# markokr/libacm

Measured on AMD Instinct MI355X. Metric: decoded PCM Msamples/sec over a batch of ACM streams (hot path on HBM-resident staged input), higher is better.
Workload: dtype int32

## Files before the change

### libacm_amd/capi.py

```python
import ctypes as C
import os

import numpy as np

from . import _build

FMT_S16LE, FMT_S16BE, FMT_U16LE, FMT_U16BE = 0, 1, 2, 3
PLAN_AUTO, PLAN_STAGEWISE = 0, 1
PLAN_FORM_ONLY, PLAN_UPLOAD_ASYNC = 0x100, 0x200
PLAN_LEAN_ALWAYS, PLAN_NO_LEAN, PLAN_FORCE_HALO, PLAN_FORCE_CARRY = 0x400, 0x800, 0x1000, 0x2000
PLAN_EXTRA = 0
BATCH_EXTRA = 0


def batch_ranges(n):
    return (int(n) & 0xFF) << 8
ERR_NO_DEVICE = -101
ERR_ARG = -103
ERR_RANGE = -105


class BlkHdr(C.Structure):
    _fields_ = [("val", C.c_uint32), ("pwr", C.c_uint32)]

# ... 394 lines not shown
    def one(i):
        if ntiles[i]:
            d = descs[i]
            buf = np.empty(cap[i], dtype=np.uint8)
            used = C.c_uint64()
            rc = L.acmhip_mform_rows(d.level, idx[d.idx_off:].ctypes.data, rows[i], buf.ctypes.data, 0, pairs[p_at[i]:].ctypes.data,
                                     C.byref(used))
            if rc == ERR_RANGE:
                ntiles[i] = 0
                return
            _check(rc, "acmhip_mform_rows")
            parts[i] = buf[:(used.value + 63) // 64 * 64]
    with ThreadPoolExecutor(max_workers=max(1, threads)) as ex:
        list(ex.map(one, range(n)))
    total = sum(p.size for p in parts if p is not None)
    if (total >> 6) >= 1 << 30:
        raise AcmHipError("byte-plane arena beyond 64 GB")
    at = 0
    for i in range(n):
        if parts[i] is not None:
            k = int(L.acmhip_mform_pairs(rows[i]))
            pairs[p_at[i]:p_at[i] + k] += np.uint32((at // 64) << 2)
            at += parts[i].size
    data = np.empty(max(at, 16) + 64, dtype=np.uint8)
    at = 0
    for i in range(n):
        if parts[i] is not None:
            data[at:at + parts[i].size] = parts[i]
            at += parts[i].size
    data[at:] = 0
    return MformArena(data, pairs, [PackedStream(p_at[i], ntiles[i], FORM_BYTEPLANE) for i in range(n)])


def mform_unrows(level, blob, pairs, nrows):
    out = np.zeros(nrows << level, dtype=np.int16)
    _check(lib().acmhip_mform_unrows(level, blob.ctypes.data, pairs.ctypes.data, nrows, out.ctypes.data), "acmhip_mform_unrows")
    return out


def pack_streams(idx, descs, threads=1):
    from concurrent.futures import ThreadPoolExecutor
    L = lib()
    n = len(descs)
    ntiles, chunk_off, blob_cap, slots = [0] * n, [0] * n, [0] * n, [0] * n
    c_at = 0
    for i, d in enumerate(descs):
        tr = L.acmhip_packed_tile_rows(d.level)
        if tr > 0 and d.row_begin == 0:
            ntiles[i] = min(d.nrows, d.n_emit >> d.level) // tr
            slots[i] = L.acmhip_packed_slots(d.level)
        chunk_off[i] = c_at
        c_at += ntiles[i] * slots[i]
        if ntiles[i]:
            mb = C.c_uint64()
            _check(L.acmhip_pack_bound(d.level, ntiles[i], C.byref(mb)), "acmhip_pack_bound")
            blob_cap[i] = (mb.value + 15) // 16 * 16
    chunks = np.zeros(max(c_at, 1), dtype=PACKED_CHUNK_DT)
    parts = [None] * n

    def one(i):
        if not ntiles[i]:
            return
        d = descs[i]
        bl = np.zeros(blob_cap[i], dtype=np.uint8)
        nb = C.c_uint64()
        _check(L.acmhip_pack_tiles(d.level, idx[d.idx_off:].ctypes.data, ntiles[i], chunks[chunk_off[i]:].ctypes.data,
# ... 364 lines not shown
```

### libacm_amd/csrc/acm_device.h

```cpp
#ifndef ACM_DEVICE_H
#define ACM_DEVICE_H

#include <stdint.h>

#include "acm_hip.h"

struct AcmDevStream {
	uint64_t idx_off;
	uint64_t hdr_off;
	uint64_t pcm_off;
	uint64_t n_emit;
	uint64_t scratch_off;
	uint32_t level;
	uint32_t rows;
	uint32_t nrows;
	uint32_t row_begin;
	uint32_t halo_row;
	uint32_t pad;
};

struct AcmTile {
	uint32_t stream;
	int32_t row0;
	uint32_t flags;
// ... 81 lines not shown
void acmhip_arena_lock(acmhip_device *dev);
void acmhip_arena_unlock(acmhip_device *dev);
int acmhip_copy_stream(acmhip_device *dev, void **out);
#define ACM_AUX_STREAMS 2
int acmhip_aux_stream(acmhip_device *dev, int k, void **out);
int acmhip_report_hip(int hip_error, const char *what);
void acmhip_set_error_text(const char *text);

#define ACMK_FMT_F32 0x100u
int acmk_tuning_build(void);
int acmk_warmup(void *stream);
int acmk_fused_variants(void);
int acmk_fused_tile_rows(uint32_t level, int variant);
int acmk_fused_has_carry(uint32_t level, int variant);
int acmk_fused_grid(uint32_t level, int variant, int cus);
int acmk_launch_fused(uint32_t level, int variant, int cus, int carry, const AcmDevStream *d_streams, const AcmTile *d_tiles,
		      uint32_t ntiles, const int16_t *d_idx, const acmhip_blkhdr *d_hdr, int16_t *d_pcm, unsigned fmt, void *stream);
int acmk_tile2_rows(uint32_t level);
int acmk_tile2_grid(uint32_t level, int cus);
#define ACM_K2_SINK_BYTES 65536
#define ACM_K2_SINK_F32_BYTES (2 * ACM_K2_SINK_BYTES)
int acmk_launch_tile2(uint32_t level, int cus, const AcmTile2 *d_tiles, uint32_t ntiles, const int16_t *d_idx, const acmhip_blkhdr *d_hdr, int16_t *d_pcm,
		      int16_t *d_sink, unsigned fmt, void *stream);
int acmk_tile2p_rows(uint32_t level);
int acmk_tile2p_group_rows(uint32_t level);
int acmk_tile2p_slots(uint32_t level);
int acmk_tile2p_waves(uint32_t level);
int acmk_tile2p_pad_shift(uint32_t level);
int acmk_launch_tile2p(uint32_t level, int cus, const AcmTile2 *d_tiles, uint32_t ntiles, const acmhip_packed_chunk *d_chunks, const uint8_t *d_blob,
		       const acmhip_blkhdr *d_hdr, int16_t *d_pcm, int16_t *d_sink, unsigned fmt, void *stream);
int acmk_tile2m_rows(uint32_t level);
int acmk_tile2m_lead_in(uint32_t level);
int acmk_tile2m_run_waves(uint32_t level, int cus);
int acmk_tile2m_grid(uint32_t level, int cus);
int acmk_tile2m_stages(uint32_t level);
int acmk_launch_tile2m(uint32_t level, int cus, const AcmTile2 *d_tiles, uint32_t ntiles, const uint8_t *d_mform, const acmhip_mform_pair *d_pairs,
		       const acmhip_blkhdr *d_hdr, int16_t *d_pcm, int16_t *d_sink, unsigned fmt, void *stream);
int acmk_launch_unpack(const AcmDevStream *d_streams, const uint32_t *d_list, uint32_t nlist, uint64_t max_elems,
		       const int16_t *d_idx, const acmhip_blkhdr *d_hdr, int32_t *d_x, uint32_t shift, void *stream);
int acmk_launch_prefix(const AcmDevStream *d_streams, const uint32_t *d_list, uint32_t nlist, uint64_t max_elems,
		       uint32_t level, const int16_t *d_idx, const acmhip_blkhdr *d_hdr, int32_t *d_y, void *stream);
int acmk_plane_tile_rows(void);
int acmk_plane_grid(int cus);
int acmk_launch_fused_plane(int cus, int carry, const AcmDevStream *d_streams, const AcmTile *d_tiles, uint32_t ntiles,
			    const int32_t *d_plane, int16_t *d_pcm, unsigned fmt, void *stream);
int acmk_launch_patch(const AcmDevPatch *d_patches, uint64_t n, int32_t *d_x, void *stream);
int acmk_launch_stage(const AcmDevStream *d_streams, const uint32_t *d_list, uint32_t nlist, uint64_t max_elems,
		      uint32_t level, uint32_t k, const int32_t *d_in, int32_t *d_out, uint32_t shift, void *stream);
int acmk_parse_supported(uint32_t level, uint32_t rows, uint64_t file_len, uint64_t blocks);
int acmk_launch_parse(const AcmParseJob *d_jobs, uint32_t njobs, const uint8_t *d_files, uint32_t *d_colpos, int16_t *d_idx,
		      acmhip_blkhdr *d_hdr, AcmParseResult *d_res, uint32_t *d_flags, uint64_t max_columns, void *stream);
#define ACM_PARSE_RANGE_MAX_STREAMS 32768
int acmk_launch_parse_range(const AcmParseJob *d_jobs, uint32_t njobs, const uint8_t *d_files, uint32_t *d_colpos, int16_t *d_idx,
			    acmhip_blkhdr *d_hdr, AcmParseResult *d_res, uint32_t *d_flags, uint64_t max_columns, uint32_t r, uint32_t R,
			    uint32_t stripes_up, void *stream);
int acmk_launch_parse_range_mf(const AcmParseJob *d_jobs, uint32_t njobs, const uint8_t *d_files, uint32_t *d_colpos, int16_t *d_idx,
			       acmhip_blkhdr *d_hdr, AcmParseResult *d_res, uint32_t *d_flags, uint64_t max_columns, uint32_t r, uint32_t R,
			       uint32_t stripes_up, uint8_t *d_mf, uint32_t *d_pairs, uint32_t *d_blkoff, void *stream);
int acmk_launch_parse_blocks(const AcmParseJob *d_jobs, uint32_t njobs, const AcmBlockJob *d_bjobs, uint32_t nblock, const uint8_t *d_files,
			     uint32_t *d_colpos, int16_t *d_idx, acmhip_blkhdr *d_hdr, AcmParseResult *d_res, uint32_t *d_flags,
			     uint64_t max_columns, void *stream);
uint32_t acmk_stripe_bound(uint32_t file_len, uint32_t s, uint32_t S);
uint32_t acmk_range_bound(uint32_t blocks, uint32_t r, uint32_t R, uint32_t unit);
int acmk_launch_scatter_stripe(const AcmParseJob *d_jobs, uint32_t njobs, const uint64_t *d_stripe_at, const uint8_t *d_stage,
			       uint8_t *d_files, uint32_t s, uint32_t S, void *stream);
int acmk_launch_small(uint32_t level, const AcmDevStream *d_streams, const uint32_t *d_list, uint32_t nlist, uint64_t max_emit,
// ... 21 lines not shown
```

### libacm_amd/csrc/acm_kernels.hip

```cpp
#include <hip/hip_runtime.h>

#include <utility>

#include "acm_device.h"

#ifndef ACM_L14_GROUPS
#define ACM_L14_GROUPS 3, 3, 3, 3, 2
#endif
#ifndef ACM_L13_GROUPS
#define ACM_L13_GROUPS 2, 3, 3, 3, 2
#endif

#ifndef ACM_OUT_F32
#define ACM_OUT_F32 0
#endif
#if ACM_OUT_F32
#define ACM_K_EMIT acm_sw_emit_f32
#define ACM_K_SMALL acm_small_level_f32
#define ACM_K_FUSED acm_fused_tile_f32
#define ACM_K_TILE2 acm_f32_tile2
#define ACM_K_CHUNK acm_f32_chunk
#define ACMK_OUT(name) name##_f32
#else
#define ACM_K_EMIT acm_sw_emit
#define ACM_K_SMALL acm_small_level
#define ACM_K_FUSED acm_fused_tile
#define ACM_K_TILE2 acm_tile2
#define ACM_K_CHUNK acm_chunk
#define ACMK_OUT(name) name
#endif

namespace {

__device__ __forceinline__ uint32_t pcm16(int32_t v, int level, unsigned fmt)
{
	uint32_t w = (uint32_t)(v >> level);
	if (fmt & 2u)
// ... 1979 lines not shown
#define ACM_K3_DPP_HISTORY 1
#endif
	static constexpr bool HISTORY_BY_DPP = ACM_K3_DPP_HISTORY && RR >= 2 && NSW == 2 && RR * SIGMA == 16 && SIGMA >= 4;
	static constexpr bool KEEPS_ROWS = HISTORY_IN_REGISTERS || HISTORY_BY_DPP;
	template <int CTRL, int BANKS>
	static __device__ __forceinline__ v4u_t dpp4(const v4u_t old, const v4u_t src)
	{
		v4u_t r;
#pragma unroll
		for (int v = 0; v < 4; v++)
			r[v] = (uint32_t)__builtin_amdgcn_update_dpp((int)old[v], (int)src[v], CTRL, 0xF, BANKS, false);
		return r;
	}
	static constexpr int DPP_W0_BANKS = (1 << (SIGMA / 4)) - 1;
	static __device__ __forceinline__ void hand_history_on(Raw &raw)
	{
#pragma unroll
		for (int k = 0; k < 2; k++) {
			raw.lo[0][k] = dpp4<0x100 + (16 - SIGMA), DPP_W0_BANKS>(raw.lo[0][k], raw.lo[0][k + NSW]);
			raw.hi[0][k] = dpp4<0x100 + (16 - SIGMA), DPP_W0_BANKS>(raw.hi[0][k], raw.hi[0][k + NSW]);
		}
	}
	static __device__ __forceinline__ void take_history_from_partner(Raw &raw)
	{
#pragma unroll
		for (int k = 0; k < 2; k++) {
			raw.lo[0][k] = dpp4<0x110 + SIGMA, 0xF & ~DPP_W0_BANKS>(raw.lo[0][k], raw.lo[0][k + NSW]);
			raw.hi[0][k] = dpp4<0x110 + SIGMA, 0xF & ~DPP_W0_BANKS>(raw.hi[0][k], raw.hi[0][k + NSW]);
		}
	}
	static constexpr int JM = (TR & 1) ? 1 : TR / 2;
	static_assert(JM + 1 <= NE, "entries in reach are entries fetched");
	static __device__ __forceinline__ uint32_t half_bytes(const uint32_t cls) { return (0x4234u >> (4u * cls)) & 15u; }
	template <int J0>
	static __device__ __forceinline__ uint32_t mode_of(const uint32_t flags, const Desc &d, const uint32_t sval)
	{
		const uint32_t cls = d.e[0] & 3u;
		const uint32_t pair_units = (uint32_t)(COLS / 64) * half_bytes(cls);
		bool ok = (flags & ACM_TILE_ONEBLOCK) != 0 && cls != 0u;
		if constexpr (OutScale<L>::SHIFT != 0)
			ok = ok && sval < 65536u;
#pragma unroll
		for (int j = 1; j <= JM; j++)
			ok = ok && (d.e[j] & 3u) == cls;
#pragma unroll
		for (int j = J0; j < JM; j++)
			ok = ok && (d.e[j + 1] >> 2) - (d.e[j] >> 2) == pair_units;
		return ok ? (cls == ACMHIP_BP_NIB12 ? 3u : cls - (ACMHIP_BP_BYTE - 1u)) : 0u;
	}

#ifndef ACM_K3_LD_MOD
#define ACM_K3_LD_MOD " nt"
#endif
	template <bool KEEP>
	static __device__ __forceinline__ void issue(Raw &raw, const uint8_t *arena, const Desc &d, const int lane, const uint32_t odd, const uint32_t mode)
	{
		static_assert(!KEEP || KEEPS_ROWS, "the rows in front belong to another lane");
		constexpr int K0 = KEEP ? 2 : 0, J0 = KEEP ? 1 : 0;
		const uint32_t i = (uint32_t)lane & 15u, ks = (uint32_t)lane >> 4;
		const uint32_t c = class_of(i), rr = RR == 1 ? 0u : i / SIGMA;
		const uint32_t smode = __builtin_amdgcn_readfirstlane(mode);
		uint32_t va[NX][NG], vh[NX][NG];
		const uint8_t *sb[NX][NG];
		if (mode) {
			const uint32_t hb = smode == 1u ? 2u : smode == 2u ? 4u : 3u;
			const uint64_t base = reinterpret_cast<uint64_t>(arena) + ((uint64_t)(d.e[J0] >> 2) << 6);
			const uint32_t vl = (rr * (uint32_t)(NSW * COLS / 2) + c * (uint32_t)(QN / 2)) * hb + 16u * ks;
			const uint32_t vlh = vl - (smode == 3u ? 8u * ks : 0u);
#pragma unroll
			for (int k = K0; k < NX; k++)
#pragma unroll
				for (int g = 0; g < NG; g++) {
					va[k][g] = vl;
					vh[k][g] = vlh;
					sb[k][g] = sgpr_u64(base + (uint64_t)((((TR & 1 ? odd : 0u) + (uint32_t)(k - K0)) * (uint32_t)(COLS / 2) + group_at(g) * (uint32_t)(QN / 2)) * hb));
				}
		} else {
			const uint32_t e0 = d.e[0];
			const uint8_t *base = sgpr_u64(reinterpret_cast<uint64_t>(arena) + ((uint64_t)(e0 >> 2) << 6));
#pragma unroll
			for (int k = K0; k < NX; k++) {
// ... 53 lines not shown
		for (int g = 0; g < NG; g++)
#pragma unroll
			for (int k = 0; k < 2; k++) {
				raw.lo[g][k] = raw.lo[g][k + NSW];
				raw.hi[g][k] = raw.hi[g][k + NSW];
			}
	}
	static __device__ __forceinline__ void zero_history(Raw &raw)
	{
		const v4u_t z = { 0, 0, 0, 0 };
#pragma unroll
		for (int g = 0; g < NG; g++)
#pragma unroll
			for (int k = 0; k < 2; k++)
				raw.lo[g][k] = raw.hi[g][k] = z;
	}

	static __device__ __forceinline__ v4i_t mfma(const v4u_t data, const v4i_t coef, const v4i_t acc)
	{
		return __builtin_amdgcn_mfma_i32_16x16x64_i8((v4i_t)data, coef, acc, 0, 0, 0);
	}

	static __device__ __forceinline__ int32_t opaque_s(int32_t v)
	{
		asm("" : "+s"(v));
		return v;
	}
	static __device__ __forceinline__ int32_t opaque_v(int32_t v)
	{
		asm("" : "+v"(v));
		return v;
	}

	template <bool WORDS, bool FAST, bool NIB = false>
	static __device__ __forceinline__ void run_t(const Raw &raw, uint32_t *const tile, const Tables &t, const int lane, const uint32_t hvs,
						     const uint32_t in_front, const uint32_t sval, const bool wordu = false, const Desc *dd = nullptr,
						     const uint32_t odd = 0u, const bool nform = false)
	{
		static_assert(!NIB || (WORDS && FAST), "rows in N form are a fast-path matter; the general path takes them to bytes first");
		const v4i_t zero = { 0, 0, 0, 0 };
		const uint32_t h = (uint32_t)lane >> 4, qd = (uint32_t)lane & 15u;
		uint32_t c0[NH], rrd[NH];
		uint32_t o_lane[NH];
#pragma unroll
		for (int hf = 0; hf < NH; hf++) {
			const uint32_t i = 4u * h + (uint32_t)(hf * NVH);
			c0[hf] = RR == 1 ? class_of(i) : i % SIGMA;
			rrd[hf] = RR == 1 ? 0u : i / SIGMA;
			const uint32_t m_lane = rrd[hf] * (uint32_t)(NSW * COLS) + c0[hf] + (uint32_t)SIGMA * qd;
			o_lane[hf] = m_lane + (m_lane >> PS);
		}
		uint32_t bias_at[NSW][NH];
		int32_t val[NSW][NH], dv2[NSW][NH], dv1[NSW][NH];
		bool step2[NSW], step1[NSW];
		bool small[NSW];
#pragma unroll
		for (int s = 0; s < NSW; s++)
			small[s] = OutScale<L>::SHIFT == 0;
		if constexpr (FAST) {
#pragma unroll
			for (int s = 0; s < NSW; s++) {
				step2[s] = step1[s] = false;
				small[s] = true;
#pragma unroll
				for (int hf = 0; hf < NH; hf++)
					val[s][hf] = dv2[s][hf] = dv1[s][hf] = 0;
			}
		} else if constexpr (RR <= 2) {
			int32_t rowval[TR + 2];
#pragma unroll
			for (int k = 0; k < TR + 2; k++)
				rowval[k] = (int32_t)__builtin_amdgcn_readlane(hvs, k);
// ... 36 lines not shown
					dv1[s][hf] = g[s] - g[s + 1];
					if (!one_val) {
						step2[s] = step2[s] || __builtin_amdgcn_ballot_w64(dv2[s][hf] != 0) != 0;
						step1[s] = step1[s] || __builtin_amdgcn_ballot_w64(dv1[s][hf] != 0) != 0;
					}
				}
			}
		}
#pragma unroll
		for (int s = 0; s < NSW; s++)
#pragma unroll
			for (int hf = 0; hf < NH; hf++) {
				const uint32_t row = in_front + rrd[hf] * NSW + s;
				bias_at[s][hf] = ((row < 2 ? row : 2u) * 2u + (c0[hf] == 0 ? 0u : 1u)) * (uint32_t)QN + qd;
			}
		const v4i_t *cf = &t.coef[0][0][lane];
		const auto &hi = raw.hi;
#ifndef ACM_K3_MT_UNROLL
#define ACM_K3_MT_UNROLL 1
#endif
#define ACM_PRAGMA_(x) _Pragma(#x)
#define ACM_UNROLL(n) ACM_PRAGMA_(unroll n)
		ACM_UNROLL(ACM_K3_MT_UNROLL)
		for (int mt = 0; mt < NM; mt++) {
			const v4i_t cf0 = cf[0], cf1 = cf[NM * 64], cf2 = cf[2 * NM * 64];
#pragma unroll
			for (int e = 0; e < NSET; e++) {
				const int g = e / NSW, s = e % NSW;
				int32_t b[NH];
#pragma unroll
				for (int hf = 0; hf < NH; hf++)
					b[hf] = g == 0 ? (&t.bias[0][0][0])[bias_at[s][hf] + 16u * (uint32_t)mt] : 0;
				const v4i_t l1 = mfma(raw.lo[g][s], cf2, zero);
				const v4i_t l2 = mfma(raw.lo[g][s + 1], cf1, l1);
				const v4i_t la = mfma(raw.lo[g][s + 2], cf0, l2);
				v4i_t y;
				if constexpr (FAST) {
					const int32_t sv = opaque_s((int32_t)__builtin_amdgcn_readfirstlane(sval));
#pragma unroll
					for (int v = 0; v < 4; v++)
						y[v] = __mul24(la[v], sv) + (v % NVH == 0 ? b[v / NVH] : 0);
					if constexpr (WORDS) {
						const v4i_t h1 = mfma(hi[g][s], cf2, zero);
						const v4i_t h2 = mfma(hi[g][s + 1], cf1, h1);
						const v4i_t ha = mfma(hi[g][s + 2], cf0, h2);
						if constexpr (NIB) {
							const int32_t sv4 = opaque_s((int32_t)__builtin_amdgcn_readfirstlane(sval << 4));
#pragma unroll
							for (int v = 0; v < 4; v++)
								y[v] = __mul24(ha[v], sv4) + y[v];
						} else {
							const uint32_t sv8 = (uint32_t)opaque_s((int32_t)__builtin_amdgcn_readfirstlane(sval << 8));
#pragma unroll
							for (int v = 0; v < 4; v++)
								y[v] = (int32_t)(__umul24((uint32_t)ha[v], sv8) + (uint32_t)y[v]);
						}
					}
				} else {
#pragma unroll
				for (int v = 0; v < 4; v++)
					y[v] = __mul24(la[v], val[s][v / NVH]) + (v % NVH == 0 ? b[v / NVH] : 0);
				if (step2[s]) {
#pragma unroll
					for (int v = 0; v < 4; v++)
						y[v] += __mul24(l2[v], dv2[s][v / NVH]);
				}
				if (step1[s]) {
#pragma unroll
					for (int v = 0; v < 4; v++)
						y[v] += __mul24(l1[v], dv1[s][v / NVH]);
// ... 47 lines not shown
					}
					if (step1[s]) {
#pragma unroll
						for (int v = 0; v < 4; v++)
							yh[v] += __mul24(h1[v], w1[v / NVH]);
					}
					const uint32_t hs = nform ? 4u : 8u;
#pragma unroll
					for (int v = 0; v < 4; v++)
						y[v] = (int32_t)(((uint32_t)opaque_v(yh[v]) << hs) + (uint32_t)y[v]);
					}
				joined:;
				}
				}
				static_assert(COLS % (1 << PS) == 0 && (SIGMA * 16) % (1 << PS) == 0 &&
					      (NG == 1 || (group_at(NG - 1) % (1 << PS) + CB + 7 < (1 << PS) && SIGMA % (1 << PS) == 0)), "address split");
#pragma unroll
				for (int hf = 0; hf < NH; hf++) {
					uint32_t *const o = tile + (o_lane[hf] + (uint32_t)((s * COLS + ((s * COLS) >> PS)) + (group_at(g) + (group_at(g) >> PS))));
#pragma unroll
					for (int v = 0; v < NVH; v++)
						o[v] = (uint32_t)y[hf * NVH + v];
				}
			}
			cf += 64;
#pragma unroll
			for (int hf = 0; hf < NH; hf++)
				o_lane[hf] += SIGMA * 16 + ((SIGMA * 16) >> PS);
		}
	}

	static __device__ __forceinline__ void run(Raw &raw, uint32_t *const tile, const Tables &t, const int lane_, const uint32_t hvs,
						   const Desc &d, const uint32_t in_front, const uint32_t odd, const uint32_t mode, const uint32_t sval,
						   const bool first)
	{
#ifdef ACM_K3_OPAQUE_LANE
		const int lane = opaque_v(lane_);
#else
		const int lane = lane_;
#endif
		const bool all_new = !KEEPS_ROWS || first;
		if (mode == 3u) {
#pragma unroll
			for (int k = 0; k < NX; k++)
				if (k >= 2 || all_new) {
#pragma unroll
					for (int g = 0; g < NG; g++)
						raw.hi[g][k] = expand_nib(raw.hi[g][k]);
				}
			if constexpr (HISTORY_BY_DPP)
				take_history_from_partner(raw);
			run_t<true, true, true>(raw, tile, t, lane, 0u, in_front, sval);
			return;
		}
		if (mode) {
			if constexpr (HISTORY_BY_DPP)
				take_history_from_partner(raw);
			if (mode == 2u)
				run_t<true, true>(raw, tile, t, lane, 0u, in_front, sval);
			else
				run_t<false, true>(raw, tile, t, lane, 0u, in_front, sval);
			return;
		}
		uint32_t any_word = 0, any_nib = 0, any_wordu = 0;
#pragma unroll
		for (int j = 0; j < NE; j++) {
			any_word |= (d.e[j] & 3u) == ACMHIP_BP_WORD ? 1u : 0u;
			any_nib |= (d.e[j] & 3u) == ACMHIP_BP_NIB12 ? 1u : 0u;
			any_wordu |= (d.e[j] & 3u) == ACMHIP_BP_WORDU ? 1u : 0u;
		}
		any_word |= any_wordu;
		const uint32_t rr = RR == 1 ? 0u : ((uint32_t)lane & 15u) / SIGMA;
		if (any_nib) {
#pragma unroll
// ... 79 lines not shown
		} else if (!(f0 & ACM_TILE_FRESH)) {
			discard = true;
			t--;
		}
	}

	auto rows_in_front = [](const AcmTile2 &r) -> uint32_t { return (r.flags & ACM_TILE_FRESH) ? 0u : (r.flags & ACM_TILE_ROW1) ? 1u : 2u; };
	auto fetch_val = [&](const AcmTile2 &r, const int lane, uint32_t v, const uint32_t mode) -> uint32_t {
		const uint32_t *p = &hdr[0].val;
		if (!mode) {
			const uint32_t lr_fetch = (uint32_t)(lane < TR + 2 ? lane : TR + 1);
			const uint32_t missing = 2u - rows_in_front(r);
			const uint32_t q = r.rowpos + (lr_fetch < missing ? 0u : lr_fetch - missing);
			const uint32_t b = r.magic ? __umulhi(q, r.magic) : q;
			p = &hdr[r.hdr_blk + b].val;
		}
		asm volatile("s_cmp_lg_u32 %2, 0\n\ts_cbranch_scc1 .Lacm_zv_%=\n\t"
			     "global_load_dword %0, %1, off\n"
			     ".Lacm_zv_%=:"
			     : "+v"(v) : "v"(p), "s"(__builtin_amdgcn_readfirstlane(mode)) : "memory", "scc");
		return v;
	};
	typedef const uint32_t __attribute__((address_space(4))) *const_u32_ptr;
	auto val_of = [&](const AcmTile2 &r) -> uint32_t {
		const uint64_t a = reinterpret_cast<uint64_t>(&hdr[__builtin_amdgcn_readfirstlane(r.hdr_blk)].val);
		return *(const_u32_ptr)a << OutScale<L>::SHIFT;
	};

	constexpr int NVEC = TR * COLS / 8, PER_OWNER = NJ_LAST / 8, NSTORE = NVEC / 64;
	static_assert(NVEC % 64 == 0, "whole rounds");
	const uint8_t *const arena = reinterpret_cast<const uint8_t *>(idx);
	auto record_at = [&](const uint32_t k) -> AcmTile2 { return tiles[__builtin_amdgcn_readfirstlane(k < t_end ? k : t_end - 1)]; };
	constexpr int MODE_J0 = FP::KEEPS_ROWS ? 1 : 0;
#ifdef ACM_K3_NO_FAST
	auto mode_of = [&](const AcmTile2 &, const typename FP::Desc &, const uint32_t) -> uint32_t { return 0u; };
#else
	auto mode_of = [&](const AcmTile2 &r, const typename FP::Desc &d, const uint32_t sval) -> uint32_t {
		return FP::template mode_of<MODE_J0>(r.flags, d, sval);
	};
#endif
	AcmTile2 cur = record_at(t);
	typename FP::Desc dcur = FP::fetch_desc(pairs, cur);
	typename FP::Raw raw;
	{
		const v4u_t z = { 0, 0, 0, 0 };
#pragma unroll
		for (int g = 0; g < FP::NG; g++)
#pragma unroll
			for (int k = 0; k < FP::NX; k++)
				raw.hi[g][k] = z;
	}
	uint32_t mode_cur = 0u, sv_cur = val_of(cur);
	uint32_t hv = fetch_val(cur, lane0, 0u, 0u);
	FP::template issue<false>(raw, arena, dcur, lane0, (cur.flags & ACM_TILE_ODD) ? 1u : 0u, 0u);
	k2_wait<0>();
	bool fresh = true, first_of_run = true;
	AcmTile2 nxt = record_at(t + 1), nx2 = record_at(t + 2);
	typename FP::Desc dnxt = FP::fetch_desc(pairs, nxt);
	uint32_t sv_nxt = val_of(nxt);
	uint32_t mode_nxt = mode_of(nxt, dnxt, sv_nxt);
#ifdef ACM_STAMPS
	unsigned long long acc_[8] = { 0, 0, 0, 0, 0, 0, 0, 0 };
	unsigned long long last_ = stamp_now();
#endif
	for (;;) {
		const uint32_t tn = t + 1;
		const bool more = tn < t_end;
		int lane = lane0;
#ifdef ACM_K3_OPAQUE_LANE
		asm volatile("" : "+v"(lane));
#endif
		if (fresh)
			for (int k = lane; k < NCARRY_WORDS; k += 64)
				carry_mem[k] = 0u;
		const uint32_t hvs = hv << OutScale<L>::SHIFT;
		ACM_STAMP(0);
		phase_prio<true, PRIO_FIRST_PASS>();
		FP::run(raw, tile, tables, lane, hvs, dcur, rows_in_front(cur), (cur.flags & ACM_TILE_ODD) ? 1u : 0u, mode_cur, sv_cur, first_of_run);
		first_of_run = false;
		phase_prio<true, PRIO_IDLE>();
		ACM_STAMP(1);

		hv = fetch_val(nxt, lane, hv, mode_nxt);
		if constexpr (FP::HISTORY_IN_REGISTERS) {
			FP::shift_history(raw);
			if (nxt.flags & ACM_TILE_FRESH)
				FP::zero_history(raw);
			FP::template issue<true>(raw, arena, dnxt, lane, (nxt.flags & ACM_TILE_ODD) ? 1u : 0u, mode_nxt);
		} else if constexpr (FP::HISTORY_BY_DPP) {
			FP::hand_history_on(raw);
			if (nxt.flags & ACM_TILE_FRESH)
				FP::zero_history(raw);
			FP::template issue<true>(raw, arena, dnxt, lane, (nxt.flags & ACM_TILE_ODD) ? 1u : 0u, mode_nxt);
		} else {
			FP::template issue<false>(raw, arena, dnxt, lane, (nxt.flags & ACM_TILE_ODD) ? 1u : 0u, mode_nxt);
		}
		const AcmTile2 nx3 = record_at(t + 3);
		const typename FP::Desc dnx2 = FP::fetch_desc(pairs, nx2);
		const uint32_t sv_nx2 = val_of(nx2);
		ACM_STAMP(2);
		phase_prio<true, PRIO_LDS_PASSES>();
		run_lds_passes<C, PASS_ABL, true, FP::G, Gs...>(tile, lane, F32 ? (unsigned)ACMHIP_FMT_S16LE : fmt, carry_mem);
		tile_barrier<MODE_WAVE>();
		ACM_STAMP(3);
		if constexpr (F32) {
			float *out = discard ? reinterpret_cast<float *>(sink) : reinterpret_cast<float *>(pcm) + cur.pcm_off;
			lean_store_f32<C, 64, NSTORE, ABL>(tile, lane, out);
		} else {
			typedef uint32_t v4u __attribute__((ext_vector_type(4)));
			v4u *out = discard ? reinterpret_cast<v4u *>(sink) : reinterpret_cast<v4u *>(reinterpret_cast<uint16_t *>(pcm) + cur.pcm_off);
#pragma unroll
			for (int k = 0; k < NSTORE; k++) {
				const int vec = lane + k * 64;
				const uint32_t *q = tile + lds_at<C::PS>((vec / PER_OWNER) * NJ_LAST) + (vec % PER_OWNER) * park_piece<NJ_LAST>();
				const v4u o = { q[0], q[1], q[2], q[3] };
#ifdef ACM_K3_ST_MOD
				asm volatile("global_store_dwordx4 %0, %1, %2" ACM_K3_ST_MOD :: "v"((uint32_t)(vec * 16)), "v"(o), "s"(sgpr_u64(reinterpret_cast<uint64_t>(out))) : "memory");
#else
				__builtin_nontemporal_store(o, &out[vec]);
#endif
			}
		}
		ACM_STAMP(5);
		phase_prio<true, PRIO_IDLE>();
		k2_wait<F32 ? 2 * NSTORE : NSTORE>();
		ACM_STAMP(6);
		tile_barrier<MODE_WAVE>();
		if (!more)
			break;
		fresh = (nxt.flags & (ACM_TILE_FRESH | ACM_TILE_DISCARD)) != 0;
		discard = (nxt.flags & ACM_TILE_DISCARD) != 0;
		cur = nxt;
		dcur = dnxt;
		sv_cur = sv_nxt;
		mode_cur = mode_nxt;
		t = tn;
		nxt = nx2;
		dnxt = dnx2;
		sv_nxt = sv_nx2;
		mode_nxt = mode_of(nxt, dnxt, sv_nxt);
		nx2 = nx3;
	}
#ifdef ACM_STAMPS
	if (lane0 == 0 && vw < 2048)
		for (int k = 0; k < 8; k++)
			g_acm_stamps[vw][k] = acc_[k];
#endif
}

struct Tile2Entry {
	typedef void (*Fn)(const AcmTile2 *, uint32_t, const int16_t *, const uint32_t *, const acmhip_blkhdr *, int16_t *, int16_t *, unsigned);
	Fn fn;
	int threads, tile_rows, wg_per_cu;
};
template <class C, int... Gs>
constexpr Tile2Entry entry_k2()
{
	return Tile2Entry{ ACM_K_TILE2<C, 4, 0, false, Gs...>, C::NT, C::TR, 1024 / C::NT };
}
template <class C, int WPC, int... Gs>
constexpr Tile2Entry entry_k2w()
{
	return Tile2Entry{ ACM_K_TILE2<C, WPC * C::NT / 256, 0, false, Gs...>, C::NT, C::TR, WPC };
}
#ifdef ACM_ABLATION
template <int ABL>
constexpr Tile2Entry abl_k2() { return Tile2Entry{ ACM_K_TILE2<TileCfg<9, 256, 8192>, 4, ABL, false, 3, 3, 3>, 256, 16, 4 }; }
const struct { int mask; Tile2Entry e; } g_tile2_abl[] = {
	{ 1, abl_k2<1>() }, { 2, abl_k2<2>() }, { 4, abl_k2<4>() }, { 6, abl_k2<6>() }, { 8, abl_k2<8>() }, { 16, abl_k2<16>() },
	{ 17, abl_k2<17>() }, { 23, abl_k2<23>() }, { 32, abl_k2<32>() }, { 25, abl_k2<25>() }, { 31, abl_k2<31>() }, { 12, abl_k2<12>() },
};
#endif
const Tile2Entry g_tile2[ACM_K2_MAX_LEVEL - ACM_K2_MIN_LEVEL + 1] = {
// ... 566 lines not shown
				e = x.e;
#endif
	uint32_t grid = (uint32_t)((cus > 0 ? cus : 256) * e.wg_per_cu);
	if (grid > ntiles)
		grid = ntiles;
	hipLaunchKernelGGL(e.fn, dim3(grid), dim3(e.threads), 0, (hipStream_t)stream, d_tiles, ntiles, d_idx, (const uint32_t *)nullptr, d_hdr, d_pcm, d_sink, fmt);
	ACMK_CHECK_LAUNCH();
	return 0;
}

#if !ACM_OUT_F32
extern "C" int acmk_tile2m_rows(uint32_t level)
{
	if (level < ACM_K2M_MIN_LEVEL || level > ACM_K2M_MAX_LEVEL)
		return 0;
	return tile2m_entry(level).e.tile_rows;
}

extern "C" int acmk_tile2m_lead_in(uint32_t level)
{
	if (level < ACM_K2M_MIN_LEVEL || level > ACM_K2M_MAX_LEVEL || tile2m_entry(level).g0 != 6)
		return 1;
	switch (level) {
	case 8: return FirstPassZ<8>::KEEPS_ROWS ? 1 + (2 + FirstPassZ<8>::NSW - 1) / FirstPassZ<8>::NSW : 1;
	case 9: return FirstPassZ<9>::KEEPS_ROWS ? 1 + (2 + FirstPassZ<9>::NSW - 1) / FirstPassZ<9>::NSW : 1;
	case 10: return FirstPassZ<10>::HISTORY_IN_REGISTERS ? 1 + (2 + FirstPassZ<10>::NSW - 1) / FirstPassZ<10>::NSW : 1;
	case 11: return FirstPassZ<11>::HISTORY_IN_REGISTERS ? 1 + (2 + FirstPassZ<11>::NSW - 1) / FirstPassZ<11>::NSW : 1;
	case 12: return FirstPassZ<12>::HISTORY_IN_REGISTERS ? 1 + (2 + FirstPassZ<12>::NSW - 1) / FirstPassZ<12>::NSW : 1;
	case 13: case 14: return 2;
	default: return 1;
	}
}

extern "C" int acmk_tile2m_run_waves(uint32_t level, int cus)
{
	if (level < ACM_K2M_MIN_LEVEL || level > 12 || tile2m_entry(level).g0 != 6)
		return 0;
	const Tile2Entry &e = tile2m_entry(level).e;
	return (cus > 0 ? cus : 256) * e.wg_per_cu * (e.threads / 64);
}

extern "C" int acmk_tile2m_grid(uint32_t level, int cus)
{
	if (level < ACM_K2M_MIN_LEVEL || level > ACM_K2M_MAX_LEVEL)
		return 0;
	return (cus > 0 ? cus : 256) * tile2m_entry(level).e.wg_per_cu;
}

extern "C" int acmk_tile2m_stages(uint32_t level)
{
	if (level < ACM_K2M_MIN_LEVEL || level > ACM_K2M_MAX_LEVEL)
		return 0;
	return tile2m_entry(level).g0;
}

#endif
extern "C" int ACMK_OUT(acmk_launch_tile2m)(uint32_t level, int cus, const AcmTile2 *d_tiles, uint32_t ntiles, const uint8_t *d_mform, const acmhip_mform_pair *d_pairs,
				  const acmhip_blkhdr *d_hdr, int16_t *d_pcm, int16_t *d_sink, unsigned fmt, void *stream)
{
#if !ACM_OUT_F32
	if (fmt & ACMK_FMT_F32)
		return acmk_launch_tile2m_f32(level, cus, d_tiles, ntiles, d_mform, d_pairs, d_hdr, d_pcm, d_sink, fmt & 3u, stream);
#endif
	if (ntiles == 0)
		return 0;
	if (!d_sink || !d_mform || !d_pairs)
// ... 118 lines not shown
```

Before: 1.347 million.

## Add fast path for tiles straddling a block boundary in tile2m first pass

Adds a boundary fast mode that lets chunks spanning two blocks take the MFMA fast path instead of the general path. The MFMA accumulation chain is split at the boundary row so each block's part is scaled by its own multiplier. The mode classification moves to a shared host/device header, and Python and host helpers are added to inspect modes. It costs an extra header load per tile and more register pressure in the first pass, and it is a correctness risk if the boundary split is wrong.

```diff
diff --git a/libacm_amd/capi.py b/libacm_amd/capi.py
--- a/libacm_amd/capi.py
+++ b/libacm_amd/capi.py
@@ -450,6 +450,64 @@
     return MformArena(data, pairs, [PackedStream(p_at[i], ntiles[i], FORM_BYTEPLANE) for i in range(n)])
 
 
+TILE2_DT = np.dtype([("idx_off", "<u8"), ("pcm_off", "<u8"), ("hdr_blk", "<u4"), ("rowpos", "<u4"), ("magic", "<u4"), ("flags", "<u4")])
+TILE_FRESH, TILE_DISCARD, TILE_ROW1, TILE_ODD, TILE_ONEBLOCK = 1, 2, 4, 8, 16
+CHUNK_BOUNDARY = 4
+_CUT_VISIT = C.CFUNCTYPE(None, C.c_void_p, C.c_char_p, C.c_uint32, C.c_void_p, C.c_size_t, C.c_size_t)
+
+
+def _chunk_mode_lib():
+    L = lib()
+    L.acmk_chunk_mode_entries.argtypes = [C.c_uint32]
+    L.acmk_chunk_boundary_fast.argtypes = [C.c_uint32]
+    L.acmk_chunk_mode.argtypes = [C.c_uint32, C.c_uint32, C.c_uint32, C.c_uint32, C.c_void_p, C.c_uint32, C.c_uint32]
+    L.acmk_chunk_modes.argtypes = [C.c_uint32, C.c_void_p, C.c_size_t, C.c_void_p, C.c_void_p, C.c_void_p]
+    L.acmk_plan_cut_visit.argtypes = [C.c_int, C.c_void_p, C.c_size_t, C.c_void_p, C.c_void_p, C.c_size_t, C.c_uint, _CUT_VISIT, C.c_void_p]
+    return L
+
+
+def chunk_mode_entries(level):
+    return _chunk_mode_lib().acmk_chunk_mode_entries(level)
+
+
+def chunk_boundary_fast(level):
+    return bool(_chunk_mode_lib().acmk_chunk_boundary_fast(level))
+
+
+def chunk_mode(level, flags, rowpos, magic, entries, val, val_next):
+    e = np.ascontiguousarray(entries, dtype=np.uint32)
+    if e.size < chunk_mode_entries(level):
+        raise ValueError("chunk_mode: %d entries, level %d looks at %d" % (e.size, level, chunk_mode_entries(level)))
+    return _chunk_mode_lib().acmk_chunk_mode(level, flags, rowpos, magic, e.ctypes.data, val, val_next)
+
+
+def chunk_records(descs, packed, cus=256, flags=0):
+    L = _chunk_mode_lib()
+    out = {}
+
+    def visit(_ctx, name, level, data, elem_bytes, count):
+        if name == b"tiles2m" and L.acmk_chunk_mode_entries(level) > 0:
+            assert elem_bytes == TILE2_DT.itemsize
+            out[level] = np.frombuffer(C.string_at(data, elem_bytes * count), dtype=TILE2_DT)
+    n = len(descs)
+    arr = (StreamDesc * max(n, 1))(*descs)
+    pk = (PackedStream * max(n, 1))(*[PackedStream(m.chunk_off, m.ntiles, m.form) for m in packed])
+    _check(L.acmk_plan_cut_visit(cus, arr, n, pk, None, 0, flags, _CUT_VISIT(visit), None), "acmk_plan_cut_visit")
+    return out
+
+
+def chunk_modes(level, records, pairs, hdr):
+    rec = np.ascontiguousarray(records, dtype=TILE2_DT)
+    pairs = np.ascontiguousarray(pairs, dtype=np.uint32)
+    hdr = np.ascontiguousarray(hdr, dtype=np.uint32).reshape(-1, 2)
+    if rec.size and (int(rec["idx_off"].max()) + chunk_mode_entries(level) > pairs.size or int(rec["hdr_blk"].max()) + 1 >= hdr.shape[0] + 1):
+        raise ValueError("chunk_modes: the records name entries or blocks beyond the tables")
+    out = np.zeros(rec.size, dtype=np.uint8)
+    if _chunk_mode_lib().acmk_chunk_modes(level, rec.ctypes.data, rec.size, pairs.ctypes.data, hdr.ctypes.data, out.ctypes.data) != 0:
+        raise ValueError("chunk_modes: level %d has no chunk kernel" % level)
+    return out
+
+
 def mform_unrows(level, blob, pairs, nrows):
     out = np.zeros(nrows << level, dtype=np.int16)
     _check(lib().acmhip_mform_unrows(level, blob.ctypes.data, pairs.ctypes.data, nrows, out.ctypes.data), "acmhip_mform_unrows")
diff --git a/libacm_amd/csrc/acm_chunk_mode.h b/libacm_amd/csrc/acm_chunk_mode.h
--- /dev/null
+++ b/libacm_amd/csrc/acm_chunk_mode.h
@@ -0,0 +1,75 @@
+#ifndef ACM_CHUNK_MODE_H
+#define ACM_CHUNK_MODE_H
+
+#include <stdint.h>
+
+#include "acm_device.h"
+
+#if defined(__HIPCC__) || defined(__CUDACC__)
+#define ACM_MODE_HD __host__ __device__ __forceinline__
+#else
+#define ACM_MODE_HD inline
+#endif
+
+#define ACM_CHUNK_BOUNDARY 4u
+#define ACM_CHUNK_BOUNDARY_VAL_LIMIT 32768u
+
+struct AcmChunkGeom {
+	uint32_t tr;
+	uint32_t jm;
+	uint32_t j0;
+	uint32_t pair_units;
+	uint32_t scaled;
+	uint32_t boundary;
+};
+
+ACM_MODE_HD uint32_t acm_chunk_half_bytes(const uint32_t cls)
+{
+	return (0x4234u >> (4u * cls)) & 15u;
+}
+
+ACM_MODE_HD uint32_t acm_chunk_load_mode(const uint32_t cls)
+{
+	return cls == ACMHIP_BP_NIB12 ? 3u : cls - (ACMHIP_BP_BYTE - 1u);
+}
+
+ACM_MODE_HD uint32_t acm_chunk_umulhi(const uint32_t a, const uint32_t b)
+{
+	return (uint32_t)(((uint64_t)a * b) >> 32);
+}
+
+template <class Entries>
+ACM_MODE_HD uint32_t acm_chunk_mode_of(const AcmChunkGeom g, const uint32_t flags, const uint32_t rowpos, const uint32_t magic, const Entries &e,
+				       const uint32_t sval, const uint32_t sval_next)
+{
+	if (flags & ACM_TILE_ONEBLOCK) {
+		const uint32_t cls = e[0] & 3u;
+		const uint32_t pair_units = g.pair_units * acm_chunk_half_bytes(cls);
+		bool ok = cls != ACMHIP_BP_WORDU;
+		if (g.scaled)
+			ok = ok && sval < 65536u;
+		for (uint32_t j = 1; j <= g.jm; j++)
+			ok = ok && (e[j] & 3u) == cls;
+		for (uint32_t j = g.j0; j < g.jm; j++)
+			ok = ok && (e[j + 1] >> 2) - (e[j] >> 2) == pair_units;
+		return ok ? acm_chunk_load_mode(cls) : 0u;
+	}
+#ifndef ACM_K3_NO_BOUNDARY_FAST
+	if (g.boundary) {
+		bool ok = (flags & (ACM_TILE_FRESH | ACM_TILE_ROW1)) == 0u && magic != 0u;
+		ok = ok && acm_chunk_umulhi(rowpos + 1u, magic) == 0u && acm_chunk_umulhi(rowpos + 2u, magic) == 1u &&
+		     acm_chunk_umulhi(rowpos + g.tr + 1u, magic) == 1u;
+		const uint32_t cls = e[1] & 3u;
+		const uint32_t pair_units = g.pair_units * acm_chunk_half_bytes(cls);
+		ok = ok && cls != ACMHIP_BP_WORDU && (e[0] & 3u) != ACMHIP_BP_WORDU;
+		for (uint32_t j = 2; j <= g.jm; j++)
+			ok = ok && (e[j] & 3u) == cls && (e[j] >> 2) - (e[j - 1] >> 2) == pair_units;
+		ok = ok && (sval | sval_next) < ACM_CHUNK_BOUNDARY_VAL_LIMIT;
+		return ok ? (ACM_CHUNK_BOUNDARY | acm_chunk_load_mode(cls)) : 0u;
+	}
+#endif
+	(void)rowpos, (void)magic, (void)sval_next;
+	return 0u;
+}
+
+#endif
diff --git a/libacm_amd/csrc/acm_device.h b/libacm_amd/csrc/acm_device.h
--- a/libacm_amd/csrc/acm_device.h
+++ b/libacm_amd/csrc/acm_device.h
@@ -137,6 +137,12 @@
 int acmk_tile2m_rows(uint32_t level);
 int acmk_tile2m_lead_in(uint32_t level);
 int acmk_tile2m_run_waves(uint32_t level, int cus);
+int acmk_chunk_mode_entries(uint32_t level);
+int acmk_chunk_boundary_fast(uint32_t level);
+int acmk_chunk_mode(uint32_t level, uint32_t flags, uint32_t rowpos, uint32_t magic, const uint32_t *entries, uint32_t val,
+		    uint32_t val_next);
+int acmk_chunk_modes(uint32_t level, const AcmTile2 *recs, size_t n, const uint32_t *pairs, const acmhip_blkhdr *hdr,
+		     uint8_t *out);
 int acmk_tile2m_grid(uint32_t level, int cus);
 int acmk_tile2m_stages(uint32_t level);
 int acmk_launch_tile2m(uint32_t level, int cus, const AcmTile2 *d_tiles, uint32_t ntiles, const uint8_t *d_mform, const acmhip_mform_pair *d_pairs,
diff --git a/libacm_amd/csrc/acm_kernels.hip b/libacm_amd/csrc/acm_kernels.hip
--- a/libacm_amd/csrc/acm_kernels.hip
+++ b/libacm_amd/csrc/acm_kernels.hip
@@ -3,6 +3,7 @@
 #include <utility>
 
 #include "acm_device.h"
+#include "acm_chunk_mode.h"
 
 #ifndef ACM_L14_GROUPS
 #define ACM_L14_GROUPS 3, 3, 3, 3, 2
@@ -2048,21 +2049,18 @@
 	static constexpr int JM = (TR & 1) ? 1 : TR / 2;
 	static_assert(JM + 1 <= NE, "entries in reach are entries fetched");
 	static __device__ __forceinline__ uint32_t half_bytes(const uint32_t cls) { return (0x4234u >> (4u * cls)) & 15u; }
+	static constexpr bool BOUNDARY_FAST = KEEPS_ROWS && NSW >= 2 && NH == 1;
 	template <int J0>
-	static __device__ __forceinline__ uint32_t mode_of(const uint32_t flags, const Desc &d, const uint32_t sval)
-	{
-		const uint32_t cls = d.e[0] & 3u;
-		const uint32_t pair_units = (uint32_t)(COLS / 64) * half_bytes(cls);
-		bool ok = (flags & ACM_TILE_ONEBLOCK) != 0 && cls != 0u;
-		if constexpr (OutScale<L>::SHIFT != 0)
-			ok = ok && sval < 65536u;
-#pragma unroll
-		for (int j = 1; j <= JM; j++)
-			ok = ok && (d.e[j] & 3u) == cls;
-#pragma unroll
-		for (int j = J0; j < JM; j++)
-			ok = ok && (d.e[j + 1] >> 2) - (d.e[j] >> 2) == pair_units;
-		return ok ? (cls == ACMHIP_BP_NIB12 ? 3u : cls - (ACMHIP_BP_BYTE - 1u)) : 0u;
+	static constexpr AcmChunkGeom geom()
+	{
+		return AcmChunkGeom{ (uint32_t)TR, (uint32_t)JM, (uint32_t)J0, (uint32_t)(COLS / 64), OutScale<L>::SHIFT != 0 ? 1u : 0u, BOUNDARY_FAST ? 1u : 0u };
+	}
+	template <int J0>
+	static __device__ __forceinline__ uint32_t mode_of(const uint32_t flags, const uint32_t rowpos, const uint32_t magic, const Desc &d, const uint32_t sval,
+							   const uint32_t sval_next)
+	{
+		static_assert(!BOUNDARY_FAST || J0 == 1, "a boundary chunk's loads start at its own first pair");
+		return acm_chunk_mode_of(geom<J0>(), flags, rowpos, magic, d.e, sval, sval_next);
 	}
 
 #ifndef ACM_K3_LD_MOD
@@ -2182,12 +2180,18 @@
 		return v;
 	}
 
-	template <bool WORDS, bool FAST, bool NIB = false>
+	struct CutMul {
+		int32_t m_new, mh_new;
+		int32_t m_old, mh_old;
+		bool words;
+	};
+	template <bool WORDS, bool FAST, bool NIB = false, bool CUT = false>
 	static __device__ __forceinline__ void run_t(const Raw &raw, uint32_t *const tile, const Tables &t, const int lane, const uint32_t hvs,
 						     const uint32_t in_front, const uint32_t sval, const bool wordu = false, const Desc *dd = nullptr,
-						     const uint32_t odd = 0u, const bool nform = false)
+						     const uint32_t odd = 0u, const bool nform = false, const CutMul cm = CutMul{ 0, 0, 0, 0, false })
 	{
 		static_assert(!NIB || (WORDS && FAST), "rows in N form are a fast-path matter; the general path takes them to bytes first");
+		static_assert(!CUT || (WORDS && FAST && !NIB && NH == 1), "the cut chains are a fast path; the form of a row is in its multiplier");
 		const v4i_t zero = { 0, 0, 0, 0 };
 		const uint32_t h = (uint32_t)lane >> 4, qd = (uint32_t)lane & 15u;
 		uint32_t c0[NH], rrd[NH];
@@ -2290,10 +2294,38 @@
 				for (int hf = 0; hf < NH; hf++)
 					b[hf] = g == 0 ? (&t.bias[0][0][0])[bias_at[s][hf] + 16u * (uint32_t)mt] : 0;
 				const v4i_t l1 = mfma(raw.lo[g][s], cf2, zero);
-				const v4i_t l2 = mfma(raw.lo[g][s + 1], cf1, l1);
-				const v4i_t la = mfma(raw.lo[g][s + 2], cf0, l2);
+				const v4i_t l2 = mfma(raw.lo[g][s + 1], cf1, CUT && s == 1 ? zero : l1);
+				const v4i_t la = mfma(raw.lo[g][s + 2], cf0, CUT && s == 0 ? zero : l2);
 				v4i_t y;
-				if constexpr (FAST) {
+				if constexpr (CUT) {
+					const int32_t mn = cm.m_new, mo = cm.m_old;
+#pragma unroll
+					for (int v = 0; v < 4; v++)
+						y[v] = __mul24(la[v], mn) + (v == 0 ? b[0] : 0);
+					{
+						if (s < 2) {
+							const v4i_t &lh = s == 0 ? l2 : l1;
+#pragma unroll
+							for (int v = 0; v < 4; v++)
+								y[v] = __mul24(lh[v], mo) + opaque_v(y[v]);
+						}
+					}
+					if (cm.words) {
+						const v4i_t h1 = mfma(hi[g][s], cf2, zero);
+						const v4i_t h2 = mfma(hi[g][s + 1], cf1, s == 1 ? zero : h1);
+						const v4i_t ha = mfma(hi[g][s + 2], cf0, s == 0 ? zero : h2);
+						const int32_t hn = cm.mh_new, ho = cm.mh_old;
+#pragma unroll
+						for (int v = 0; v < 4; v++)
+							y[v] = __mul24(ha[v], hn) + opaque_v(y[v]);
+						if (s < 2) {
+							const v4i_t &hh = s == 0 ? h2 : h1;
+#pragma unroll
+							for (int v = 0; v < 4; v++)
+								y[v] = __mul24(hh[v], ho) + opaque_v(y[v]);
+						}
+					}
+				} else if constexpr (FAST) {
 					const int32_t sv = opaque_s((int32_t)__builtin_amdgcn_readfirstlane(sval));
 #pragma unroll
 					for (int v = 0; v < 4; v++)
@@ -2407,7 +2439,7 @@
 
 	static __device__ __forceinline__ void run(Raw &raw, uint32_t *const tile, const Tables &t, const int lane_, const uint32_t hvs,
 						   const Desc &d, const uint32_t in_front, const uint32_t odd, const uint32_t mode, const uint32_t sval,
-						   const bool first)
+						   const bool first, const uint32_t sval_next = 0u)
 	{
 #ifdef ACM_K3_OPAQUE_LANE
 		const int lane = opaque_v(lane_);
@@ -2415,6 +2447,31 @@
 		const int lane = lane_;
 #endif
 		const bool all_new = !KEEPS_ROWS || first;
+		if constexpr (BOUNDARY_FAST) {
+			if (mode & ACM_CHUNK_BOUNDARY) {
+				const uint32_t own = mode & 3u, front = d.e[0] & 3u;
+				if (own == 3u) {
+#pragma unroll
+					for (int k = 2; k < NX; k++)
+#pragma unroll
+						for (int g = 0; g < NG; g++)
+							raw.hi[g][k] = expand_nib(raw.hi[g][k]);
+				}
+				if constexpr (HISTORY_BY_DPP)
+					take_history_from_partner(raw);
+				CutMul cm;
+				const uint32_t sn = __builtin_amdgcn_readfirstlane(sval_next), so = __builtin_amdgcn_readfirstlane(sval);
+				cm.m_new = opaque_s((int32_t)sn);
+				cm.mh_new = opaque_s(own == 1u ? 0 : (int32_t)(sn << (own == 2u ? 8u : 4u)));
+				const int32_t mh_front = front == ACMHIP_BP_BYTE ? 0 : (int32_t)(so << (front == ACMHIP_BP_WORD ? 8u : 4u));
+				const bool w0 = RR == 1 || (4u * ((uint32_t)lane >> 4)) / SIGMA == 0u;
+				cm.m_old = opaque_v(w0 ? (int32_t)so : (int32_t)sn);
+				cm.mh_old = opaque_v(w0 ? mh_front : (own == 1u ? 0 : (int32_t)(sn << (own == 2u ? 8u : 4u))));
+				cm.words = !(own == 1u && front == ACMHIP_BP_BYTE);
+				run_t<true, true, false, true>(raw, tile, t, lane, 0u, in_front, 0u, false, nullptr, 0u, false, cm);
+				return;
+			}
+		}
 		if (mode == 3u) {
 #pragma unroll
 			for (int k = 0; k < NX; k++)
@@ -2560,11 +2617,20 @@
 	const uint8_t *const arena = reinterpret_cast<const uint8_t *>(idx);
 	auto record_at = [&](const uint32_t k) -> AcmTile2 { return tiles[__builtin_amdgcn_readfirstlane(k < t_end ? k : t_end - 1)]; };
 	constexpr int MODE_J0 = FP::KEEPS_ROWS ? 1 : 0;
+	auto val_next_of = [&](const AcmTile2 &r) -> uint32_t {
+		if constexpr (FP::BOUNDARY_FAST) {
+			const uint32_t b = __builtin_amdgcn_readfirstlane(r.hdr_blk) + ((r.flags & ACM_TILE_ONEBLOCK) ? 0u : 1u);
+			const uint64_t a = reinterpret_cast<uint64_t>(&hdr[b].val);
+			return *(const_u32_ptr)a << OutScale<L>::SHIFT;
+		} else {
+			return 0u;
+		}
+	};
 #ifdef ACM_K3_NO_FAST
-	auto mode_of = [&](const AcmTile2 &, const typename FP::Desc &, const uint32_t) -> uint32_t { return 0u; };
+	auto mode_of = [&](const AcmTile2 &, const typename FP::Desc &, const uint32_t, const uint32_t) -> uint32_t { return 0u; };
 #else
-	auto mode_of = [&](const AcmTile2 &r, const typename FP::Desc &d, const uint32_t sval) -> uint32_t {
-		return FP::template mode_of<MODE_J0>(r.flags, d, sval);
+	auto mode_of = [&](const AcmTile2 &r, const typename FP::Desc &d, const uint32_t sval, const uint32_t sval_next) -> uint32_t {
+		return FP::template mode_of<MODE_J0>(r.flags, r.rowpos, r.magic, d, sval, sval_next);
 	};
 #endif
 	AcmTile2 cur = record_at(t);
@@ -2578,15 +2644,15 @@
 			for (int k = 0; k < FP::NX; k++)
 				raw.hi[g][k] = z;
 	}
-	uint32_t mode_cur = 0u, sv_cur = val_of(cur);
+	uint32_t mode_cur = 0u, sv_cur = val_of(cur), sw_cur = 0u;
 	uint32_t hv = fetch_val(cur, lane0, 0u, 0u);
 	FP::template issue<false>(raw, arena, dcur, lane0, (cur.flags & ACM_TILE_ODD) ? 1u : 0u, 0u);
 	k2_wait<0>();
 	bool fresh = true, first_of_run = true;
 	AcmTile2 nxt = record_at(t + 1), nx2 = record_at(t + 2);
 	typename FP::Desc dnxt = FP::fetch_desc(pairs, nxt);
-	uint32_t sv_nxt = val_of(nxt);
-	uint32_t mode_nxt = mode_of(nxt, dnxt, sv_nxt);
+	uint32_t sv_nxt = val_of(nxt), sw_nxt = val_next_of(nxt);
+	uint32_t mode_nxt = mode_of(nxt, dnxt, sv_nxt, sw_nxt);
 #ifdef ACM_STAMPS
 	unsigned long long acc_[8] = { 0, 0, 0, 0, 0, 0, 0, 0 };
 	unsigned long long last_ = stamp_now();
@@ -2604,7 +2670,7 @@
 		const uint32_t hvs = hv << OutScale<L>::SHIFT;
 		ACM_STAMP(0);
 		phase_prio<true, PRIO_FIRST_PASS>();
-		FP::run(raw, tile, tables, lane, hvs, dcur, rows_in_front(cur), (cur.flags & ACM_TILE_ODD) ? 1u : 0u, mode_cur, sv_cur, first_of_run);
+		FP::run(raw, tile, tables, lane, hvs, dcur, rows_in_front(cur), (cur.flags & ACM_TILE_ODD) ? 1u : 0u, mode_cur, sv_cur, first_of_run, sw_cur);
 		first_of_run = false;
 		phase_prio<true, PRIO_IDLE>();
 		ACM_STAMP(1);
@@ -2614,18 +2680,18 @@
 			FP::shift_history(raw);
 			if (nxt.flags & ACM_TILE_FRESH)
 				FP::zero_history(raw);
-			FP::template issue<true>(raw, arena, dnxt, lane, (nxt.flags & ACM_TILE_ODD) ? 1u : 0u, mode_nxt);
+			FP::template issue<true>(raw, arena, dnxt, lane, (nxt.flags & ACM_TILE_ODD) ? 1u : 0u, mode_nxt & 3u);
 		} else if constexpr (FP::HISTORY_BY_DPP) {
 			FP::hand_history_on(raw);
 			if (nxt.flags & ACM_TILE_FRESH)
 				FP::zero_history(raw);
-			FP::template issue<true>(raw, arena, dnxt, lane, (nxt.flags & ACM_TILE_ODD) ? 1u : 0u, mode_nxt);
+			FP::template issue<true>(raw, arena, dnxt, lane, (nxt.flags & ACM_TILE_ODD) ? 1u : 0u, mode_nxt & 3u);
 		} else {
-			FP::template issue<false>(raw, arena, dnxt, lane, (nxt.flags & ACM_TILE_ODD) ? 1u : 0u, mode_nxt);
+			FP::template issue<false>(raw, arena, dnxt, lane, (nxt.flags & ACM_TILE_ODD) ? 1u : 0u, mode_nxt & 3u);
 		}
 		const AcmTile2 nx3 = record_at(t + 3);
 		const typename FP::Desc dnx2 = FP::fetch_desc(pairs, nx2);
-		const uint32_t sv_nx2 = val_of(nx2);
+		const uint32_t sv_nx2 = val_of(nx2), sw_nx2 = val_next_of(nx2);
 		ACM_STAMP(2);
 		phase_prio<true, PRIO_LDS_PASSES>();
 		run_lds_passes<C, PASS_ABL, true, FP::G, Gs...>(tile, lane, F32 ? (unsigned)ACMHIP_FMT_S16LE : fmt, carry_mem);
@@ -2661,12 +2727,14 @@
 		cur = nxt;
 		dcur = dnxt;
 		sv_cur = sv_nxt;
+		sw_cur = sw_nxt;
 		mode_cur = mode_nxt;
 		t = tn;
 		nxt = nx2;
 		dnxt = dnx2;
 		sv_nxt = sv_nx2;
-		mode_nxt = mode_of(nxt, dnxt, sv_nxt);
+		sw_nxt = sw_nx2;
+		mode_nxt = mode_of(nxt, dnxt, sv_nxt, sw_nxt);
 		nx2 = nx3;
 	}
 #ifdef ACM_STAMPS
@@ -3299,6 +3367,67 @@
 	}
 }
 
+template <int L>
+static int chunk_mode_host(uint32_t flags, uint32_t rowpos, uint32_t magic, const uint32_t *entries, uint32_t val, uint32_t val_next)
+{
+	using FP = FirstPassZ<L>;
+	return (int)acm_chunk_mode_of(FP::template geom<FP::KEEPS_ROWS ? 1 : 0>(), flags, rowpos, magic, entries, val << OutScale<L>::SHIFT,
+				      val_next << OutScale<L>::SHIFT);
+}
+extern "C" int acmk_chunk_mode_entries(uint32_t level)
+{
+	if (level < 8 || level > 12 || tile2m_entry(level).g0 != 6)
+		return 0;
+	switch (level) {
+	case 8: return FirstPassZ<8>::JM + 1;
+	case 9: return FirstPassZ<9>::JM + 1;
+	case 10: return FirstPassZ<10>::JM + 1;
+	case 11: return FirstPassZ<11>::JM + 1;
+	default: return FirstPassZ<12>::JM + 1;
+	}
+}
+extern "C" int acmk_chunk_boundary_fast(uint32_t level)
+{
+#ifdef ACM_K3_NO_BOUNDARY_FAST
+	(void)level;
+	return 0;
+#else
+	if (acmk_chunk_mode_entries(level) <= 0)
+		return 0;
+	switch (level) {
+	case 8: return FirstPassZ<8>::BOUNDARY_FAST;
+	case 9: return FirstPassZ<9>::BOUNDARY_FAST;
+	case 10: return FirstPassZ<10>::BOUNDARY_FAST;
+	case 11: return FirstPassZ<11>::BOUNDARY_FAST;
+	default: return FirstPassZ<12>::BOUNDARY_FAST;
+	}
+#endif
+}
+extern "C" int acmk_chunk_mode(uint32_t level, uint32_t flags, uint32_t rowpos, uint32_t magic, const uint32_t *entries, uint32_t val, uint32_t val_next)
+{
+	if (level < 8 || level > 12 || tile2m_entry(level).g0 != 6 || !entries)
+		return -1;
+	switch (level) {
+	case 8: return chunk_mode_host<8>(flags, rowpos, magic, entries, val, val_next);
+	case 9: return chunk_mode_host<9>(flags, rowpos, magic, entries, val, val_next);
+	case 10: return chunk_mode_host<10>(flags, rowpos, magic, entries, val, val_next);
+	case 11: return chunk_mode_host<11>(flags, rowpos, magic, entries, val, val_next);
+	default: return chunk_mode_host<12>(flags, rowpos, magic, entries, val, val_next);
+	}
+}
+
+extern "C" int acmk_chunk_modes(uint32_t level, const AcmTile2 *recs, size_t n, const uint32_t *pairs, const acmhip_blkhdr *hdr, uint8_t *out)
+{
+	if (acmk_chunk_mode_entries(level) <= 0 || !recs || !pairs || !hdr || !out)
+		return -1;
+	for (size_t k = 0; k < n; k++) {
+		const AcmTile2 &r = recs[k];
+		const uint32_t next = (r.flags & ACM_TILE_ONEBLOCK) ? 0u : 1u;
+		out[k] = (uint8_t)acmk_chunk_mode(level, r.flags, r.rowpos, r.magic, pairs + r.idx_off, hdr[r.hdr_blk].val, hdr[r.hdr_blk + next].val);
+	}
+	return 0;
+}
+
 extern "C" int acmk_tile2m_run_waves(uint32_t level, int cus)
 {
 	if (level < ACM_K2M_MIN_LEVEL || level > 12 || tile2m_entry(level).g0 != 6)
diff --git a/profiles/chunk_mode_breakdown.py b/profiles/chunk_mode_breakdown.py
--- /dev/null
+++ b/profiles/chunk_mode_breakdown.py
@@ -0,0 +1,50 @@
+#!/usr/bin/env python3
+import argparse
+import json
+import os
+import sys
+
+ROOT = os.path.dirname(os.path.dirname(os.path.abspath(__file__)))
+sys.path.insert(0, ROOT)
+
+import numpy as np
+
+
+def main():
+    ap = argparse.ArgumentParser()
+    ap.add_argument("--level", type=int, default=9)
+    ap.add_argument("--rows", type=int, default=16)
+    ap.add_argument("--blocks", type=int, default=250)
+    ap.add_argument("--streams", type=int, default=16)
+    ap.add_argument("--cus", type=int, default=256)
+    a = ap.parse_args()
+    from libacm_amd import capi, workload
+    threads = max(4, min(64, workload.usable_cpus()))
+    b = workload.build_uniform(a.streams, a.level, a.rows, a.blocks, threads=threads)
+    mf = capi.mform_streams(b.idx, b.descs, threads=threads)
+    recs = capi.chunk_records(b.descs, mf.streams, cus=a.cus)[a.level]
+    modes = capi.chunk_modes(a.level, recs, mf.pairs, b.hdr)
+    n = capi.chunk_mode_entries(a.level)
+    cls = np.stack([mf.pairs[recs["idx_off"].astype(np.int64) + j] & 3 for j in range(n)], axis=1)
+    general = modes == 0
+    oneblock = (recs["flags"] & capi.TILE_ONEBLOCK) != 0
+    first = (recs["flags"] & (capi.TILE_FRESH | capi.TILE_ROW1)) != 0
+    own_uniform = (cls[:, 1:] == cls[:, 1:2]).all(axis=1)
+    out = {
+        "level": a.level, "rows": a.rows, "blocks": a.blocks, "streams": a.streams, "records": int(recs.size),
+        "modes": {str(m): int((modes == m).sum()) for m in np.unique(modes)},
+        "boundary_path_share": round(float(((modes & capi.CHUNK_BOUNDARY) != 0).mean()), 5),
+        "general_share": round(float(general.mean()), 5),
+        "general_inside_one_block_share": round(float((general & oneblock).mean()), 5),
+        "general_at_a_boundary_share": round(float((general & ~oneblock).mean()), 5),
+        "general_at_a_boundary_own_pairs_of_two_widths_share": round(float((general & ~oneblock & ~own_uniform).mean()), 5),
+        "general_first_rows_of_a_stream_share": round(float((general & first).mean()), 5),
+        "records_without_oneblock_share": round(float((~oneblock).mean()), 5),
+        "boundary_combinations_front_own": {"%d/%d" % (f, o): int((((modes & capi.CHUNK_BOUNDARY) != 0) & (cls[:, 0] == f) & (cls[:, 1] == o)).sum())
+                                            for f in (1, 2, 3) for o in (1, 2, 3)},
+    }
+    print(json.dumps(out))
+
+
+if __name__ == "__main__":
+    main()
```

Measured after the change: 1.355 million, median of 3. No clear change (+0.6%).
